# kezakool/flair-for-aigle

Hardware: AMD Instinct MI355X
Metric: 512x512x5 tiles/sec (train fwd+bwd+AdamW), U-Net ResNet-34, 19 classes (higher is better)
Workload: dtype bf16; 1 GPU; synthetic 512x512x5 tiles, 19-class U-Net (ResNet-34 encoder), batch 32 per GPU, train step (BASELINE.json configs[1]); global_batch=32, tile=512, parallelism=dp1

## Files before the change

flair-for-aigle_amd/csrc/conv_wgrad.hip:

```cpp
#include "ffa_gfx950.h"
#include "conv_call.h"

#include <stdlib.h>

#ifndef FFA_WGRAD_TRACE
#define FFA_WGRAD_TRACE 0
#endif
#if FFA_WGRAD_TRACE
__device__ long long ffa_wgrad_trace_buf[64 * 256];
#define FFA_WTRACE(slot_)                                                                   \
  if (trace_on) {                                                                           \
    if (trace_n < 256)                                                                      \
      ffa_wgrad_trace_buf[(blockIdx.y * gridDim.x + blockIdx.x) * 256 + trace_n] =          \
          (long long)(slot_) << 56 | (__builtin_readcyclecounter() & 0xFFFFFFFFFFFFFFLL);    \
    ++trace_n;                                                                              \
  }
#else
#define FFA_WTRACE(slot_)
#endif

struct WgradArgs {
  const void* x;
  const void* dy;
  float* slabs;
// ... 765 lines not shown
    }
  }
  float* mine = sh + (sl * NQ + ql) * ROW;
#pragma unroll
  for (int t = 0; t < TAPS; ++t)
#pragma unroll
    for (int e = 0; e < 4; ++e) mine[t * 4 + e] = acc[t][e];
  __syncthreads();
  const int ci_lo = q0 * 4;
  const int nci = min(NQ * 4, Ci - ci_lo);
  float* dst = dw + ((size_t)co * Ci + ci_lo) * TAPS;
  for (int o = threadIdx.x; o < nci * TAPS; o += 256) {
    const int cl = o / TAPS, tap = o % TAPS;
    const float* col = sh + (cl >> 2) * ROW + tap * 4 + (cl & 3);
    float t = 0.f;
#pragma unroll 8
    for (int l = 0; l < SL; ++l) t += col[l * NQ * ROW];
    dst[o] = accumulate ? (dst[o] + t) : t;
  }
}


template <int CI, int CO>
struct WgThinGeom {
  static constexpr int TH = 8, TW = 32;
  static constexpr int IH = TH + 2, IW = TW + 2;
  static constexpr int XB = CI * 2, YB = CO * 2;
  static constexpr int XP = IH * IW * (XB / 16);
  static constexpr int YP = TH * TW * (YB / 16);
  static constexpr int PIECES = XP + YP;
  static constexpr int NHW = (PIECES + 255) / 256;
  static constexpr int X_BYTES = XP * 16;
  static constexpr int SLOT = PIECES * 16;
  static constexpr int NSLOT = (3 * SLOT <= 78 * 1024) ? 3 : 2;
  static constexpr int MT = CO / 16, NT = CI / 16;
  static constexpr int ACC_BYTES = MT * NT * 9 * 4 * 64 * 4;
  static constexpr int LDS_BYTES = (NSLOT * SLOT > 2 * ACC_BYTES) ? NSLOT * SLOT : 2 * ACC_BYTES;
  static_assert(2 * LDS_BYTES <= 160 * 1024, "two blocks per CU");
};

template <int CI, int CO, bool UP, bool PRO = false>
__global__ void __launch_bounds__(256, 2) conv3x3_thin_wgrad_kernel(WgradArgs a) {
  using G = WgThinGeom<CI, CO>;
  constexpr int MT = G::MT, NT = G::NT;
  __shared__ __align__(16) unsigned char smem[G::LDS_BYTES];

  const int tid = threadIdx.x;
  const int lane = tid & 63;
  const int wave = __builtin_amdgcn_readfirstlane(tid >> 6);
  const int li = lane & 15;
  const int kg = lane >> 4;

  int pinfo[G::NHW];
#pragma unroll
  for (int k = 0; k < G::NHW; ++k) {
    const int p = tid + k * 256;
    if (p < G::XP) {
      const int q = p / (G::XB / 16), sl = p % (G::XB / 16);
      pinfo[k] = ((((q / G::IW) << 8) | (q % G::IW)) << 4) | sl;
    } else if (p < G::PIECES) {
      const int j = p - G::XP;
      const int q = j / (G::YB / 16), sl = j % (G::YB / 16);
      pinfo[k] = (1 << 30) | ((((q / G::TW) << 8) | (q % G::TW)) << 4) | sl;
    } else {
      pinfo[k] = -1;
    }
  }
  const unsigned char* x_b = static_cast<const unsigned char*>(a.x);
  const unsigned char* dy_b = static_cast<const unsigned char*>(a.dy);
  const unsigned char* zero = reinterpret_cast<const unsigned char*>(ffa_zero16);
  const int Hs = UP ? (a.Hi >> 1) : a.Hi, Ws = UP ? (a.Wi >> 1) : a.Wi;
  const bool has_tail = (G::PIECES % 256 == 0) || (wave * 64 + (G::NHW - 1) * 256 < G::PIECES);

  auto tile_origin = [&](int t, int& b, int& oy0, int& ox0) {
    const int tx = t % a.tiles_x;
    const int t2 = t / a.tiles_x;
    oy0 = (t2 % a.tiles_y) * G::TH;
    b = t2 / a.tiles_y;
    ox0 = tx * G::TW;
  };
  auto issue_tile = [&](int t, int slot) {
    int b, oy0, ox0;
    tile_origin(t, b, oy0, ox0);
#pragma unroll
    for (int k = 0; k < G::NHW; ++k) {
      const int info = pinfo[k];
      const int yy = (info >> 12) & 0xff, xx = (info >> 4) & 0xff, sl = info & 15;
      const unsigned char* src = zero;
      if (info >= 0) {
        if (info & (1 << 30)) {
          const int oy = oy0 + yy, ox = ox0 + xx;
          if (oy < a.Ho && ox < a.Wo) src = dy_b + ((size_t)((b * a.Ho + oy) * a.Wo + ox) * G::YB + sl * 16);
        } else {
          const int vy = oy0 - 1 + yy, vx = ox0 - 1 + xx;
          if (vy >= 0 && vx >= 0 && vy < a.Hi && vx < a.Wi) {
            const int sy = UP ? (vy >> 1) : vy, sx = UP ? (vx >> 1) : vx;
            src = x_b + ((size_t)((b * Hs + sy) * Ws + sx) * G::XB + sl * 16);
          }
        }
      }
      const unsigned dst = (unsigned)(size_t)(__attribute__((address_space(3))) void*)(
          smem + slot * G::SLOT + (wave * 64 + k * 256) * 16);
      if (k + 1 < G::NHW || G::PIECES % 256 == 0) {
        ffa_lds_dma16(src, dst);
      } else if (has_tail) {
        if (info >= 0) ffa_lds_dma16(src, dst);
      }
    }
  };
  auto fix_tile = [&](int t, int slot) {
    if constexpr (PRO) {
      int b, oy0, ox0;
      tile_origin(t, b, oy0, ox0);
      float sc[8], sh[8];
      const int c0 = (tid % (G::XB / 16)) * 8;
      ffa_load8<float>(a.pro_sc + c0, sc);
      ffa_load8<float>(a.pro_sh + c0, sh);
#pragma unroll
      for (int k = 0; k < G::NHW; ++k) {
        const int info = pinfo[k];
        const int yy = (info >> 12) & 0xff, xx = (info >> 4) & 0xff;
        const int vy = oy0 - 1 + yy, vx = ox0 - 1 + xx;
        if (info >= 0 && !(info & (1 << 30)) && vy >= 0 && vx >= 0 && vy < a.Hi && vx < a.Wi) {
          ffa_u32x4* ptr = reinterpret_cast<ffa_u32x4*>(smem + slot * G::SLOT + (tid + k * 256) * 16);
          ffa_u32x4 v = *ptr;
          float f[8];
          f[0] = __uint_as_float(v.x << 16); f[1] = __uint_as_float(v.x & 0xffff0000u);
          f[2] = __uint_as_float(v.y << 16); f[3] = __uint_as_float(v.y & 0xffff0000u);
          f[4] = __uint_as_float(v.z << 16); f[5] = __uint_as_float(v.z & 0xffff0000u);
          f[6] = __uint_as_float(v.w << 16); f[7] = __uint_as_float(v.w & 0xffff0000u);
#pragma unroll
          for (int e = 0; e < 8; ++e) f[e] = fmaxf(__builtin_fmaf(f[e], sc[e], sh[e]), 0.f);
          v.x = ffa_pack_bf16x2(f[0], f[1]);
          v.y = ffa_pack_bf16x2(f[2], f[3]);
          v.z = ffa_pack_bf16x2(f[4], f[5]);
          v.w = ffa_pack_bf16x2(f[6], f[7]);
          *ptr = v;
        }
      }
    }
  };
  auto wait_tile = [&](int t, int slot) {
    if constexpr (PRO) {
      if constexpr (G::NSLOT == 3) {
        if (has_tail) ffa_wait_vm<G::NHW>();
        else ffa_wait_vm<G::NHW - 1>();
      } else {
        ffa_wait_vm<0>();
      }
      fix_tile(t, slot);
      ffa_wait_lgkm_barrier();
    } else if constexpr (G::NSLOT == 3) {
      if (has_tail) ffa_wait_vm_barrier<G::NHW>();
      else ffa_wait_vm_barrier<G::NHW - 1>();
    } else {
      ffa_wait_vm_barrier<0>();
    }
  };

  ffa_f32x4 acc[MT][NT][9];
#pragma unroll
  for (int mt = 0; mt < MT; ++mt)
#pragma unroll
    for (int nt = 0; nt < NT; ++nt)
#pragma unroll
      for (int tp = 0; tp < 9; ++tp) acc[mt][nt][tp] = ffa_f32x4{0.f, 0.f, 0.f, 0.f};

  const int px0 = 8 * kg + (li >> 2);
  const int aBase = G::X_BYTES + ((2 * wave) * G::TW + px0) * G::YB + (li & 3) * 8;
  const int bBase = ((2 * wave) * G::IW + px0) * G::XB + (li & 3) * 8;

  auto tr2 = [&](const unsigned char* p0, int step) {
    const ffa_s16x4 v0 = ffa_lds_read_tr16(p0);
    const ffa_s16x4 v1 = ffa_lds_read_tr16(p0 + step);
    ffa_u32x4 f;
    f.x = __builtin_bit_cast(ffa_u32x2, v0).x;
    f.y = __builtin_bit_cast(ffa_u32x2, v0).y;
    f.z = __builtin_bit_cast(ffa_u32x2, v1).x;
    f.w = __builtin_bit_cast(ffa_u32x2, v1).y;
    return f;
  };

  int t = blockIdx.x;
  const int stride = gridDim.x;
  if (t < a.npt) {
    issue_tile(t, 0);
    if constexpr (G::NSLOT == 3) issue_tile(t + stride < a.npt ? t + stride : t, 1);
    int slot = 0;
    for (; t < a.npt; t += stride) {
      wait_tile(t, slot);
      {
        const int tn = t + (G::NSLOT - 1) * stride;
        issue_tile(tn < a.npt ? tn : t, (slot + G::NSLOT - 1) % G::NSLOT);
      }
      const unsigned char* sS = smem + slot * G::SLOT;
#pragma unroll
      for (int rr = 0; rr < 2; ++rr) {
        ffa_u32x4 af[MT];
#pragma unroll
        for (int mt = 0; mt < MT; ++mt) af[mt] = tr2(sS + aBase + rr * G::TW * G::YB + mt * 32, 4 * G::YB);
#pragma unroll
        for (int tp = 0; tp < 9; ++tp) {
#pragma unroll
          for (int nt = 0; nt < NT; ++nt) {
            const ffa_u32x4 bf = tr2(sS + bBase + ((rr + tp / 3) * G::IW + tp % 3) * G::XB + nt * 32, 4 * G::XB);
#pragma unroll
            for (int mt = 0; mt < MT; ++mt)
              acc[mt][nt][tp] = __builtin_amdgcn_mfma_f32_16x16x32_bf16(__builtin_bit_cast(ffa_bf16x8, af[mt]),
                                                                       __builtin_bit_cast(ffa_bf16x8, bf), acc[mt][nt][tp],
                                                                       0, 0, 0);
          }
        }
      }
      slot = (slot + 1) % G::NSLOT;
    }
  }
  ffa_wait_vm_barrier<0>();

  float* red = reinterpret_cast<float*>(smem);
  constexpr int NACC = MT * NT * 9 * 4;
  auto put = [&](int which) {
    float* dst = red + (size_t)which * NACC * 64 + lane;
    int o = 0;
#pragma unroll
    for (int mt = 0; mt < MT; ++mt)
#pragma unroll
      for (int nt = 0; nt < NT; ++nt)
#pragma unroll
        for (int tp = 0; tp < 9; ++tp)
#pragma unroll
          for (int i = 0; i < 4; ++i) dst[(o++) * 64] = acc[mt][nt][tp][i];
  };
  auto add = [&](int which) {
    const float* src = red + (size_t)which * NACC * 64 + lane;
    int o = 0;
#pragma unroll
    for (int mt = 0; mt < MT; ++mt)
#pragma unroll
      for (int nt = 0; nt < NT; ++nt)
#pragma unroll
        for (int tp = 0; tp < 9; ++tp)
#pragma unroll
          for (int i = 0; i < 4; ++i) acc[mt][nt][tp][i] += src[(o++) * 64];
  };
  if (wave >= 2) put(wave - 2);
  __syncthreads();
  if (wave < 2) add(wave);
  __syncthreads();
  if (wave == 1) put(0);
  __syncthreads();
  if (wave != 0) return;
  add(0);

  float* slab = a.slabs + (size_t)blockIdx.x * a.CoT * 9 * a.CiT;
#pragma unroll
  for (int mt = 0; mt < MT; ++mt)
#pragma unroll
    for (int nt = 0; nt < NT; ++nt)
#pragma unroll
      for (int tp = 0; tp < 9; ++tp)
#pragma unroll
        for (int i = 0; i < 4; ++i) {
          const int co = mt * 16 + 4 * kg + i, ci = nt * 16 + li;
          slab[((size_t)co * 9 + tp) * a.CiT + ci] = acc[mt][nt][tp][i];
        }
}


template <int TW_>
struct Wg64Geom {
  static constexpr int TW = TW_, TH = 256 / TW_, IH = TH + 2, IW = TW + 2;
  static constexpr int RS = 32 / TW;
  static constexpr int XP = IH * IW * 8, YP = TH * TW * 8;
  static constexpr int PIECES = XP + YP;
  static constexpr int NHW = (PIECES + 511) / 512;
  static constexpr int X_BYTES = XP * 16;
  static constexpr int SLOT = PIECES * 16;
  static constexpr int ACC_BYTES = 144 * 64 * 4;
  static constexpr int LDS_BYTES = (2 * SLOT > 4 * ACC_BYTES) ? 2 * SLOT : 4 * ACC_BYTES;
  static_assert(TW == 32 || TW == 16, "tile width");
  static_assert(LDS_BYTES <= 160 * 1024, "LDS budget");
};

__device__ __forceinline__ int wg64_phi(int px) { return ((px >> 1) & 1) | (((px >> 3) & 1) << 1); }

template <int TW>
__global__ void __launch_bounds__(512) conv3x3_wgrad64_kernel(WgradArgs a) {
  using G = Wg64Geom<TW>;
  __shared__ __align__(16) unsigned char smem[G::LDS_BYTES];
  const int tid = threadIdx.x;
  const int lane = tid & 63;
  const int wave = __builtin_amdgcn_readfirstlane(tid >> 6);
  const int kgp = wave >> 2;
  const int wco = (wave >> 1) & 1, wci = wave & 1;
  const int li = lane & 15, kg = lane >> 4;
  const int cib = blockIdx.x % a.ncib, cob = blockIdx.x / a.ncib;
  const int co0 = cob * 64, ci0 = cib * 64;
  const int split = blockIdx.y;

  const bool two = a.C1 > 0;
  const bool from_lo = two && ci0 < a.C1;
  const size_t xpb = (size_t)(!two ? a.Ci : from_lo ? a.C1 : a.Ci - a.C1) * 2, ypb = (size_t)a.Co * 2;
  const int xW = from_lo ? a.Wi / 2 : a.Wi, xH = from_lo ? a.Hi / 2 : a.Hi;
  int pinfo[G::NHW];
#pragma unroll
  for (int k = 0; k < G::NHW; ++k) {
    const int p = tid + k * 512;
    if (p < G::XP) {
      const int q = p >> 3, yy = q / G::IW, xx = q % G::IW, sl = (p & 7) ^ (2 * wg64_phi(xx));
      const int py = from_lo ? ((yy - 1) >> 1) + 1 : yy, px = from_lo ? ((xx - 1) >> 1) + 1 : xx;
      pinfo[k] = ((((py * xW + px) * (int)xpb) >> 4) + sl) << 13 | (yy << 6) | xx;
    } else if (p < G::PIECES) {
      const int q = (p - G::XP) >> 3, yy = q / G::TW, xx = q % G::TW, sl = (p & 7) ^ (2 * wg64_phi(xx));
      pinfo[k] = ((((yy * a.Wo + xx) * (int)ypb) >> 4) + sl) << 13 | (1 << 12) | (yy << 6) | xx;
    } else {
      pinfo[k] = 1 << 11;
    }
  }
  const unsigned char* x_b = (two && !from_lo) ? static_cast<const unsigned char*>(a.x2) + (ci0 - a.C1) * 2
                                               : static_cast<const unsigned char*>(a.x) + ci0 * 2;
  const unsigned char* dy_b = static_cast<const unsigned char*>(a.dy) + co0 * 2;
  const unsigned char* zero = reinterpret_cast<const unsigned char*>(ffa_zero16);
  const bool has_tail = (G::PIECES % 512 == 0) || (wave * 64 + (G::NHW - 1) * 512 < G::PIECES);

  auto tile_origin = [&](int t, int& b, int& oy0, int& ox0) {
    const int tx = t % a.tiles_x;
    const int t2 = t / a.tiles_x;
    oy0 = (t2 % a.tiles_y) * G::TH;
    b = t2 / a.tiles_y;
    ox0 = tx * G::TW;
  };
  auto issue_tile = [&](int t, int slot) {
    int b, oy0, ox0;
    tile_origin(t, b, oy0, ox0);
    const int xoy = from_lo ? (oy0 >> 1) - 1 : oy0 - 1, xox = from_lo ? (ox0 >> 1) - 1 : ox0 - 1;
    const unsigned char* xt = x_b + ((long long)(b * xH + xoy) * xW + xox) * (long long)xpb;
    const unsigned char* yt = dy_b + ((long long)(b * a.Ho + oy0) * a.Wo + ox0) * (long long)ypb;
#pragma unroll
    for (int k = 0; k < G::NHW; ++k) {
      const int info = pinfo[k];
      const int yy = (info >> 6) & 31, xx = info & 63;
      const bool mixed = (k == G::XP / 512) && (G::XP % 512 != 0);
      const bool is_dy = mixed ? (info & (1 << 12)) != 0 : (k * 512 >= G::XP);
      const int oy = yy + (is_dy ? oy0 : oy0 - 1), ox = xx + (is_dy ? ox0 : ox0 - 1);
      const bool valid = (unsigned)oy < (unsigned)a.Ho && (unsigned)ox < (unsigned)a.Wo;
      const unsigned char* src = valid ? (is_dy ? yt : xt) + (size_t)(((unsigned)info >> 13) << 4) : zero;
      const unsigned dst = (unsigned)(size_t)(__attribute__((address_space(3))) void*)(
          smem + slot * G::SLOT + (wave * 64 + k * 512) * 16);
      if (k + 1 < G::NHW || G::PIECES % 512 == 0) {
        ffa_lds_dma16(src, dst);
      } else if (has_tail) {
        if (!(info & (1 << 11))) ffa_lds_dma16(src, dst);
      }
      __builtin_amdgcn_sched_barrier(0);
    }
  };

  ffa_f32x4 acc[2][2][9];
#pragma unroll
  for (int mt = 0; mt < 2; ++mt)
#pragma unroll
    for (int nt = 0; nt < 2; ++nt)
#pragma unroll
      for (int tp = 0; tp < 9; ++tp) acc[mt][nt][tp] = ffa_f32x4{0.f, 0.f, 0.f, 0.f};

  const int kpx = 8 * kg + (li >> 2);
  const int seg = (li & 1) * 8, hbit = (li >> 1) & 1;
  const int yphi = wg64_phi(kpx % G::TW);
  int aoff[2];
#pragma unroll
  for (int mt = 0; mt < 2; ++mt)
    aoff[mt] = G::X_BYTES + (kgp * 128 + kpx) * 128 + (((2 * (wco * 2 + mt) + hbit) ^ (2 * yphi)) * 16) + seg;

  int boff[3][2][2];
#pragma unroll
  for (int sx = 0; sx < 3; ++sx)
#pragma unroll
    for (int nt = 0; nt < 2; ++nt)
#pragma unroll
      for (int h = 0; h < 2; ++h) {
        const int hx = kpx % G::TW + sx + 4 * h;
        boff[sx][nt][h] = ((kpx / G::TW) * G::IW + hx) * 128 + (((2 * (wci * 2 + nt) + hbit) ^ (2 * wg64_phi(hx))) * 16) + seg;
      }
  auto tr2 = [&](const unsigned char* p0, const unsigned char* p1) {
    const ffa_s16x4 v0 = ffa_lds_read_tr16(p0);
    const ffa_s16x4 v1 = ffa_lds_read_tr16(p1);
    ffa_u32x4 f;
    f.x = __builtin_bit_cast(ffa_u32x2, v0).x;
    f.y = __builtin_bit_cast(ffa_u32x2, v0).y;
    f.z = __builtin_bit_cast(ffa_u32x2, v1).x;
    f.w = __builtin_bit_cast(ffa_u32x2, v1).y;
    return f;
  };

  const int ntl = (a.npt - split + a.nsplit - 1) / a.nsplit;
  if (ntl > 0) {
    issue_tile(split, 0);
    int slot = 0;
    for (int it = 0; it < ntl; ++it) {
      ffa_wait_vm_barrier<0>();
      const bool more = it + 1 < ntl;
      if (more) issue_tile(split + (it + 1) * a.nsplit, slot ^ 1);
      const unsigned char* sS = smem + slot * G::SLOT;
      ffa_u32x4 af[4][2];
      const unsigned char* sRow = sS + (G::RS * 4 * kgp) * (G::IW * 128);
#pragma unroll
      for (int hr = 0; hr < G::RS * 3 + 3; ++hr) {
        if (hr % G::RS == 0 && hr / G::RS < 4) {
#pragma unroll
          for (int mt = 0; mt < 2; ++mt)
            af[hr / G::RS][mt] = tr2(sS + aoff[mt] + (hr / G::RS) * 32 * 128, sS + aoff[mt] + (hr / G::RS) * 32 * 128 + 4 * 128);
        }
#pragma unroll
        for (int sx = 0; sx < 3; ++sx) {
#pragma unroll
          for (int nt = 0; nt < 2; ++nt) {
            const ffa_u32x4 bf = tr2(sRow + hr * (G::IW * 128) + boff[sx][nt][0], sRow + hr * (G::IW * 128) + boff[sx][nt][1]);
#pragma unroll
            for (int r = 0; r < 3; ++r) {
              if (hr - r < 0 || (hr - r) % G::RS != 0 || (hr - r) / G::RS > 3) continue;
              const int rr = (hr - r) / G::RS;
#pragma unroll
              for (int mt = 0; mt < 2; ++mt)
                acc[mt][nt][r * 3 + sx] = __builtin_amdgcn_mfma_f32_16x16x32_bf16(
                    __builtin_bit_cast(ffa_bf16x8, af[rr][mt]), __builtin_bit_cast(ffa_bf16x8, bf), acc[mt][nt][r * 3 + sx], 0, 0,
                    0);
            }
          }
        }
        __builtin_amdgcn_sched_barrier(0);
      }
      slot ^= 1;
    }
  }
  ffa_wait_vm_barrier<0>();

  float* red = reinterpret_cast<float*>(smem) + (size_t)(wave & 3) * 144 * 64 + lane;
  if (kgp == 1) {
    int o = 0;
#pragma unroll
    for (int mt = 0; mt < 2; ++mt)
#pragma unroll
      for (int nt = 0; nt < 2; ++nt)
#pragma unroll
        for (int tp = 0; tp < 9; ++tp)
#pragma unroll
          for (int i = 0; i < 4; ++i) red[(o++) * 64] = acc[mt][nt][tp][i];
  }
  __syncthreads();
  if (kgp == 1) return;
  {
    int o = 0;
#pragma unroll
    for (int mt = 0; mt < 2; ++mt)
#pragma unroll
      for (int nt = 0; nt < 2; ++nt)
#pragma unroll
        for (int tp = 0; tp < 9; ++tp)
#pragma unroll
          for (int i = 0; i < 4; ++i) acc[mt][nt][tp][i] += red[(o++) * 64];
  }
  float* slab = a.slabs + (size_t)split * a.CoT * 9 * a.CiT;
#pragma unroll
  for (int mt = 0; mt < 2; ++mt)
#pragma unroll
    for (int nt = 0; nt < 2; ++nt)
#pragma unroll
      for (int tp = 0; tp < 9; ++tp)
#pragma unroll
        for (int i = 0; i < 4; ++i) {
          const int co = co0 + wco * 32 + mt * 16 + 4 * kg + i, ci = ci0 + wci * 32 + nt * 16 + li;
          slab[((size_t)co * 9 + tp) * a.CiT + ci] = acc[mt][nt][tp][i];
        }
}


struct WgStem8Geom {
  static constexpr int TH = 8, TW = 32, IH = 2 * TH + 5, IWC = 72;
  static constexpr int XP = IH * IWC, YP = TH * TW * 8;
  static constexpr int PIECES = XP + YP;
  static constexpr int NHW = (PIECES + 511) / 512;
  static constexpr int X_BYTES = XP * 16;
  static constexpr int SLOT = PIECES * 16;
  static constexpr int ACC_BYTES = 112 * 64 * 4;
  static constexpr int LDS_BYTES = (2 * SLOT > 4 * ACC_BYTES) ? 2 * SLOT : 4 * ACC_BYTES;
  static_assert(LDS_BYTES <= 160 * 1024, "LDS budget");
};

__global__ void __launch_bounds__(512) stem_wgrad8_kernel(WgradArgs a) {
  using G = WgStem8Geom;
  __shared__ __align__(16) unsigned char smem[G::LDS_BYTES];
  const int tid = threadIdx.x;
  const int lane = tid & 63;
  const int wave = __builtin_amdgcn_readfirstlane(tid >> 6);
  const int kgp = wave >> 2;
  const int sp = wave & 3;
  const int li = lane & 15, kg = lane >> 4;
  const int split = blockIdx.y;

  int pinfo[G::NHW];
#pragma unroll
  for (int k = 0; k < G::NHW; ++k) {
    const int p = tid + k * 512;
    if (p < G::XP) {
      const int hy = p / G::IWC, hx = p % G::IWC;
      pinfo[k] = (hx < 2 * G::TW + 5) ? (((hy * a.Wi + hx) * 2) << 14 | (hy << 7) | hx) : (1 << 12);
    } else if (p < G::PIECES) {
      const int q = (p - G::XP) >> 3, yy = q / G::TW, xx = q % G::TW, sl = (p & 7) ^ (2 * wg64_phi(xx));
      pinfo[k] = ((yy * a.Wo + xx) * 8 + sl) << 14 | (1 << 13) | (yy << 7) | xx;
    } else {
      pinfo[k] = 1 << 12;
    }
  }
  const unsigned char* x_b = static_cast<const unsigned char*>(a.x);
  const unsigned char* dy_b = static_cast<const unsigned char*>(a.dy);
  const unsigned char* zero = reinterpret_cast<const unsigned char*>(ffa_zero16);
  const bool has_tail = (G::PIECES % 512 == 0) || (wave * 64 + (G::NHW - 1) * 512 < G::PIECES);
  const int tiles_x = (a.Wo + G::TW - 1) / G::TW, tiles_y = (a.Ho + G::TH - 1) / G::TH;
  const int npt = a.B * tiles_x * tiles_y;

  auto issue_tile = [&](int t, int slot) {
    const int tx = t % tiles_x, t2 = t / tiles_x;
    const int oy0 = (t2 % tiles_y) * G::TH, b = t2 / tiles_y, ox0 = tx * G::TW;
    const int iy0 = 2 * oy0 - 3, ix0 = 2 * ox0 - 3;
    const unsigned char* xt = x_b + ((long long)(b * a.Hi + iy0) * a.Wi + ix0) * 32;
    const unsigned char* yt = dy_b + ((long long)(b * a.Ho + oy0) * a.Wo + ox0) * 128;
#pragma unroll
    for (int k = 0; k < G::NHW; ++k) {
      const int info = pinfo[k];
      const int yy = (info >> 7) & 31, xx = info & 127;
      const bool mixed = (k == G::XP / 512) && (G::XP % 512 != 0);
      const bool is_dy = mixed ? (info & (1 << 13)) != 0 : (k * 512 >= G::XP);
      const bool valid = !(info & (1 << 12)) &&
                         (is_dy ? (oy0 + yy < a.Ho && ox0 + xx < a.Wo)
                                : ((unsigned)(iy0 + yy) < (unsigned)a.Hi && (unsigned)(ix0 + xx) < (unsigned)a.Wi));
      const unsigned char* src = valid ? (is_dy ? yt : xt) + (size_t)(((unsigned)info >> 14) << 4) : zero;
      const unsigned dst = (unsigned)(size_t)(__attribute__((address_space(3))) void*)(
          smem + slot * G::SLOT + (wave * 64 + k * 512) * 16);
      if (k + 1 < G::NHW || G::PIECES % 512 == 0) {
        ffa_lds_dma16(src, dst);
      } else if (has_tail) {
        if (tid + k * 512 < G::PIECES) ffa_lds_dma16(src, dst);
      }
      __builtin_amdgcn_sched_barrier(0);
    }
  };

  ffa_f32x4 acc[4][7];
#pragma unroll
  for (int mt = 0; mt < 4; ++mt)
#pragma unroll
    for (int r = 0; r < 7; ++r) acc[mt][r] = ffa_f32x4{0.f, 0.f, 0.f, 0.f};

  const int kpx = 8 * kg + (li >> 2);
  const int seg = (li & 1) * 8, hbit = (li >> 1) & 1;
  const int yphi = wg64_phi(kpx);
  int aoff[4];
#pragma unroll
  for (int mt = 0; mt < 4; ++mt)
    aoff[mt] = G::X_BYTES + (kgp * 128 + kpx) * 128 + (((2 * mt + hbit) ^ (2 * yphi)) * 16) + seg;
  const int boff = ((2 * 4 * kgp) * G::IWC + 2 * kpx + 2 * sp) * 16 + (li & 3) * 8;

  auto tr2 = [&](const unsigned char* p0, int step) {
    const ffa_s16x4 v0 = ffa_lds_read_tr16(p0);
    const ffa_s16x4 v1 = ffa_lds_read_tr16(p0 + step);
    ffa_u32x4 f;
    f.x = __builtin_bit_cast(ffa_u32x2, v0).x;
    f.y = __builtin_bit_cast(ffa_u32x2, v0).y;
    f.z = __builtin_bit_cast(ffa_u32x2, v1).x;
    f.w = __builtin_bit_cast(ffa_u32x2, v1).y;
    return f;
  };

  const int ntl = (npt - split + a.nsplit - 1) / a.nsplit;
  if (ntl > 0) {
    issue_tile(split, 0);
    int slot = 0;
    for (int it = 0; it < ntl; ++it) {
      ffa_wait_vm_barrier<0>();
      if (it + 1 < ntl) issue_tile(split + (it + 1) * a.nsplit, slot ^ 1);
      const unsigned char* sS = smem + slot * G::SLOT;
      ffa_u32x4 af[4][4];
#pragma unroll
      for (int j = 0; j < 4; ++j)
#pragma unroll
        for (int mt = 0; mt < 4; ++mt) af[j][mt] = tr2(sS + aoff[mt] + j * 32 * 128, 4 * 128);
#pragma unroll
      for (int h = 0; h < 13; ++h) {
        const ffa_u32x4 bf = tr2(sS + boff + h * (G::IWC * 16), 4 * 2 * 16);
#pragma unroll
        for (int j = 0; j < 4; ++j) {
          const int r = h - 2 * j;
          if (r < 0 || r > 6) continue;
#pragma unroll
          for (int mt = 0; mt < 4; ++mt)
            acc[mt][r] = __builtin_amdgcn_mfma_f32_16x16x32_bf16(__builtin_bit_cast(ffa_bf16x8, af[j][mt]),
                                                                 __builtin_bit_cast(ffa_bf16x8, bf), acc[mt][r], 0, 0, 0);
        }
      }
      slot ^= 1;
    }
  }
  ffa_wait_vm_barrier<0>();

  float* red = reinterpret_cast<float*>(smem) + (size_t)(wave & 3) * 112 * 64 + lane;
  if (kgp == 1) {
    int o = 0;
#pragma unroll
    for (int mt = 0; mt < 4; ++mt)
#pragma unroll
      for (int r = 0; r < 7; ++r)
#pragma unroll
        for (int i = 0; i < 4; ++i) red[(o++) * 64] = acc[mt][r][i];
  }
  __syncthreads();
  if (kgp == 1) return;
  {
    int o = 0;
#pragma unroll
    for (int mt = 0; mt < 4; ++mt)
#pragma unroll
      for (int r = 0; r < 7; ++r)
#pragma unroll
        for (int i = 0; i < 4; ++i) acc[mt][r][i] += red[(o++) * 64];
  }
  const int s = 2 * sp + (li >> 3), ch = li & 7;
  if (s < 7) {
#pragma unroll
    for (int mt = 0; mt < 4; ++mt)
#pragma unroll
      for (int r = 0; r < 7; ++r)
#pragma unroll
        for (int i = 0; i < 4; ++i) {
          const int co = mt * 16 + 4 * kg + i;
          a.slabs[(((size_t)split * a.CoT + co) * 49 + r * 7 + s) * 16 + ch] = acc[mt][r][i];
        }
  }
}


struct WgradPlan {
  int wco, wci, wk, th, tw, rg, nsplit, ncob, ncib, CoT, CiT, npt, tiles_x, tiles_y, ring, nslab, stem, thin;
};

static bool wgrad_plan(int dtype, int kh, int kw, int stride, int Co, int Ci, int B, int Ho, int Wo, WgradPlan* p,
                       bool allow_ring = true, bool allow_thin = true) {
  const bool s1 = (kh == 3 && kw == 3 && stride == 1);
  const bool s2 = (kh == 3 && kw == 3 && stride == 2);
  const bool one = (kh == 1 && kw == 1 && (stride == 1 || stride == 2));
  const bool stem = (kh == 7 && kw == 7 && stride == 2);
  if (!(s1 || s2 || one || stem)) return false;
  const bool f32 = (dtype == FFA_F32);
  p->rg = stem ? 1 : kh;
  p->wk = 1;
  p->thin = 0;
  {
    const char* tw_ = getenv("FFA_THIN_WGRAD");
    if (allow_thin && s1 && !f32 && !(tw_ && tw_[0] == '0') && (Co == 16 || Co == 32) && (Ci == 16 || Ci == 32)) {
      p->thin = 1;
      p->th = 8; p->tw = 32;
      p->wco = p->wci = 1;
      p->ncob = p->ncib = 1;
      p->CoT = Co; p->CiT = Ci;
      p->tiles_x = ffa_cdiv(Wo, 32);
      p->tiles_y = ffa_cdiv(Ho, 8);
      p->npt = B * p->tiles_x * p->tiles_y;
      p->ring = 0; p->stem = 0;
      p->nsplit = p->npt < 512 ? p->npt : 512;
      p->nslab = p->nsplit;
      return true;
    }
  }
  if (s1) {
    p->tw = (Wo >= 32) ? 32 : 16;
    p->th = (Wo >= 32) ? 4 : 8;
    p->wco = (Co > 32) ? 2 : 1;
    p->wci = (Ci > 32 && !f32) ? 2 : 1;
    if (!f32) {
      p->wk = 4 / (p->wco * p->wci);
      if (p->wk == 1) {
        p->wk = 2;
        p->th *= 2;
      } else if (p->wk == 4) {
        static const bool small_tiles = getenv("FFA_WG_THIN_SMALL") && getenv("FFA_WG_THIN_SMALL")[0] == '1';
        if (!small_tiles) p->th *= 2;
      }
    }
  } else {
    p->tw = 16;
    p->th = stem ? 8 : 4;
    p->wco = 2;
    p->wci = (f32 || stem) ? 1 : 2;
    if (stem && !f32) p->wk = 2;
  }
  p->stem = (stem && !f32 && Ci <= 16 && Co % 64 == 0) ? 1 : 0;
  p->ncob = ffa_cdiv(Co, 32 * p->wco);
  p->ncib = ffa_cdiv(Ci, 32 * p->wci);
  p->CoT = p->ncob * 32 * p->wco;
  p->CiT = p->ncib * 32 * p->wci;
  p->tiles_x = ffa_cdiv(Wo, p->tw);
  p->tiles_y = ffa_cdiv(Ho, p->th);
  p->npt = B * p->tiles_x * p->tiles_y;
  const int tile_blocks = p->ncob * p->ncib * (kh / p->rg);
  static const bool ring_enabled = getenv("FFA_WGRAD_RING") && getenv("FFA_WGRAD_RING")[0] == '1';
  const int ring_th = p->th / 2;
  p->ring = (ring_enabled && allow_ring && s1 && !f32 && p->wco == 2 && p->wci == 2 && p->wk == 2 && Ho % ring_th == 0 &&
             Wo % p->tw == 0 && (long long)B * Ho * Wo * (Co > Ci ? Co : Ci) * 2 < (1LL << 31))
                ? 1
                : 0;
  if (p->ring) {
    p->th = ring_th;
    p->wk = 1;
    p->tiles_y = ffa_cdiv(Ho, p->th);
    p->npt = B * p->tiles_x * p->tiles_y;
  }
  const int threads = 64 * p->wco * p->wci * p->wk;
  int ns = (p->ring || threads >= 512) ? 256 / tile_blocks : ffa_cdiv(512, tile_blocks);
  if (ns > p->npt) ns = p->npt;
  if (ns < 1) ns = 1;
  if (p->stem) {
    p->wk = 1;
    p->CoT = Co;
    p->CiT = 16;
    ns = 256 / (Co / 64);
    if (ns > p->npt) ns = p->npt;
    if (ns < 1) ns = 1;
  }
  p->nsplit = ns;
  const bool merge = p->wk > 1 && (p->wco * p->wci == 4 || stem);
  p->nslab = merge ? ns : ns * p->wk;
  return true;
// ... 290 lines not shown
```

Before: 2411 tiles/s.

## Software-pipeline LDS fragment reads in wgrad64 and precompute edge-validity masks

The 64-channel 3x3 wgrad kernel's inner loop is flattened into a single step sequence, with B-fragment LDS transposed reads prefetched three steps ahead in a small register queue. The A-fragment read is also issued early, before it is needed, so LDS latency overlaps the MFMA chain. Separately, per-piece bounds checks in the tile-issue path are replaced by precomputed edge bitmasks ANDed with a per-tile edge mask, removing per-piece coordinate arithmetic. The prefetch queue raises register pressure, and the mask scheme assumes only the first and last tiles can touch borders.

After: 2412 tiles/s (median of 3 runs). About the same (+0.1%).

```diff
diff --git a/flair-for-aigle_amd/csrc/conv_wgrad.hip b/flair-for-aigle_amd/csrc/conv_wgrad.hip
--- a/flair-for-aigle_amd/csrc/conv_wgrad.hip
+++ b/flair-for-aigle_amd/csrc/conv_wgrad.hip
@@ -1091,6 +1091,7 @@
   const bool from_lo = two && ci0 < a.C1;
   const size_t xpb = (size_t)(!two ? a.Ci : from_lo ? a.C1 : a.Ci - a.C1) * 2, ypb = (size_t)a.Co * 2;
   const int xW = from_lo ? a.Wi / 2 : a.Wi, xH = from_lo ? a.Hi / 2 : a.Hi;
+  const int ylast = (a.tiles_y - 1) * G::TH, xlast = (a.tiles_x - 1) * G::TW;
   int pinfo[G::NHW];
 #pragma unroll
   for (int k = 0; k < G::NHW; ++k) {
@@ -1098,10 +1099,12 @@
     if (p < G::XP) {
       const int q = p >> 3, yy = q / G::IW, xx = q % G::IW, sl = (p & 7) ^ (2 * wg64_phi(xx));
       const int py = from_lo ? ((yy - 1) >> 1) + 1 : yy, px = from_lo ? ((xx - 1) >> 1) + 1 : xx;
-      pinfo[k] = ((((py * xW + px) * (int)xpb) >> 4) + sl) << 13 | (yy << 6) | xx;
+      const int edge = (yy == 0 ? 1 : 0) | (yy - 1 + ylast >= a.Ho ? 2 : 0) | (xx == 0 ? 4 : 0) | (xx - 1 + xlast >= a.Wo ? 8 : 0);
+      pinfo[k] = ((((py * xW + px) * (int)xpb) >> 4) + sl) << 13 | edge;
     } else if (p < G::PIECES) {
       const int q = (p - G::XP) >> 3, yy = q / G::TW, xx = q % G::TW, sl = (p & 7) ^ (2 * wg64_phi(xx));
-      pinfo[k] = ((((yy * a.Wo + xx) * (int)ypb) >> 4) + sl) << 13 | (1 << 12) | (yy << 6) | xx;
+      const int edge = (yy + ylast >= a.Ho ? 2 : 0) | (xx + xlast >= a.Wo ? 8 : 0);
+      pinfo[k] = ((((yy * a.Wo + xx) * (int)ypb) >> 4) + sl) << 13 | (1 << 12) | edge;
     } else {
       pinfo[k] = 1 << 11;
     }
@@ -1125,14 +1128,13 @@
     const int xoy = from_lo ? (oy0 >> 1) - 1 : oy0 - 1, xox = from_lo ? (ox0 >> 1) - 1 : ox0 - 1;
     const unsigned char* xt = x_b + ((long long)(b * xH + xoy) * xW + xox) * (long long)xpb;
     const unsigned char* yt = dy_b + ((long long)(b * a.Ho + oy0) * a.Wo + ox0) * (long long)ypb;
+    const int tile_edge = (oy0 == 0 ? 1 : 0) | (oy0 == ylast ? 2 : 0) | (ox0 == 0 ? 4 : 0) | (ox0 == xlast ? 8 : 0);
 #pragma unroll
     for (int k = 0; k < G::NHW; ++k) {
       const int info = pinfo[k];
-      const int yy = (info >> 6) & 31, xx = info & 63;
       const bool mixed = (k == G::XP / 512) && (G::XP % 512 != 0);
       const bool is_dy = mixed ? (info & (1 << 12)) != 0 : (k * 512 >= G::XP);
-      const int oy = yy + (is_dy ? oy0 : oy0 - 1), ox = xx + (is_dy ? ox0 : ox0 - 1);
-      const bool valid = (unsigned)oy < (unsigned)a.Ho && (unsigned)ox < (unsigned)a.Wo;
+      const bool valid = (info & tile_edge) == 0;
       const unsigned char* src = valid ? (is_dy ? yt : xt) + (size_t)(((unsigned)info >> 13) << 4) : zero;
       const unsigned dst = (unsigned)(size_t)(__attribute__((address_space(3))) void*)(
           smem + slot * G::SLOT + (wave * 64 + k * 512) * 16);
@@ -1193,29 +1195,35 @@
       const unsigned char* sS = smem + slot * G::SLOT;
       ffa_u32x4 af[4][2];
       const unsigned char* sRow = sS + (G::RS * 4 * kgp) * (G::IW * 128);
-#pragma unroll
-      for (int hr = 0; hr < G::RS * 3 + 3; ++hr) {
-        if (hr % G::RS == 0 && hr / G::RS < 4) {
+      constexpr int PF = 3, NHR = G::RS * 3 + 3, NS = NHR * 6;
+      auto bf_read = [&](int s) {
+        const int hr = s / 6, sx = (s / 2) % 3, nt = s & 1;
+        return tr2(sRow + hr * (G::IW * 128) + boff[sx][nt][0], sRow + hr * (G::IW * 128) + boff[sx][nt][1]);
+      };
+      auto af_read = [&](int j) {
+#pragma unroll
+        for (int mt = 0; mt < 2; ++mt)
+          af[j][mt] = tr2(sS + aoff[mt] + j * 32 * 128, sS + aoff[mt] + j * 32 * 128 + 4 * 128);
+      };
+      ffa_u32x4 bq[PF];
+      af_read(0);
+#pragma unroll
+      for (int s = 0; s < PF; ++s) bq[s] = bf_read(s);
+      __builtin_amdgcn_sched_barrier(0);
+#pragma unroll
+      for (int s = 0; s < NS; ++s) {
+        const int hr = s / 6, sx = (s / 2) % 3, nt = s & 1;
+        const ffa_u32x4 bf = bq[s % PF];
+        if (s + PF < NS) bq[s % PF] = bf_read(s + PF);
+        if (s % 6 == 2 && (hr + 1) % G::RS == 0 && (hr + 1) / G::RS < 4) af_read((hr + 1) / G::RS);
+#pragma unroll
+        for (int r = 0; r < 3; ++r) {
+          if (hr - r < 0 || (hr - r) % G::RS != 0 || (hr - r) / G::RS > 3) continue;
+          const int rr = (hr - r) / G::RS;
 #pragma unroll
           for (int mt = 0; mt < 2; ++mt)
-            af[hr / G::RS][mt] = tr2(sS + aoff[mt] + (hr / G::RS) * 32 * 128, sS + aoff[mt] + (hr / G::RS) * 32 * 128 + 4 * 128);
-        }
-#pragma unroll
-        for (int sx = 0; sx < 3; ++sx) {
-#pragma unroll
-          for (int nt = 0; nt < 2; ++nt) {
-            const ffa_u32x4 bf = tr2(sRow + hr * (G::IW * 128) + boff[sx][nt][0], sRow + hr * (G::IW * 128) + boff[sx][nt][1]);
-#pragma unroll
-            for (int r = 0; r < 3; ++r) {
-              if (hr - r < 0 || (hr - r) % G::RS != 0 || (hr - r) / G::RS > 3) continue;
-              const int rr = (hr - r) / G::RS;
-#pragma unroll
-              for (int mt = 0; mt < 2; ++mt)
-                acc[mt][nt][r * 3 + sx] = __builtin_amdgcn_mfma_f32_16x16x32_bf16(
-                    __builtin_bit_cast(ffa_bf16x8, af[rr][mt]), __builtin_bit_cast(ffa_bf16x8, bf), acc[mt][nt][r * 3 + sx], 0, 0,
-                    0);
-            }
-          }
+            acc[mt][nt][r * 3 + sx] = __builtin_amdgcn_mfma_f32_16x16x32_bf16(
+                __builtin_bit_cast(ffa_bf16x8, af[rr][mt]), __builtin_bit_cast(ffa_bf16x8, bf), acc[mt][nt][r * 3 + sx], 0, 0, 0);
         }
         __builtin_amdgcn_sched_barrier(0);
       }
```
